# KTH-RPL/cloth-splatting

Measured on AMD Instinct MI355X. Metric: rasterizer fwd+bwd rendered Mpix/s (scene_1, 800x800), higher is better.
Workload: dtype f32

## Files before the change

cloth-splatting_amd/csrc/csplat_raster.hip:

```cpp
#include "csplat_common.h"

#include <atomic>
#include <cstring>
#include <chrono>
#include <mutex>
#include <type_traits>

#include "csplat_raster_math.h"
#include "csplat_raster_k1.h"
#include "csplat_raster_binning.h"
#include "csplat_raster_k5b_k6.h"

namespace {

constexpr int ACC_STRIDE = 16;

#define CSPLAT_ROWMASK_OP(OP, dst, src0, src1, RM)                                                                                  \
    asm("s_nop 1\n\tv_" OP "_f32_dpp %0, %1, %2 quad_perm:[0,1,2,3] row_mask:" RM " bank_mask:0xf" : "+v"(dst) : "v"(src0), "v"(src1))
__device__ __forceinline__ void rows_scan_mul(float f, float Tin, float &Tr, float &Tout) {
    const auto s16 = __builtin_amdgcn_permlane16_swap(__float_as_uint(f), __float_as_uint(f), false, false);
    const float ev = __uint_as_float(s16[0]), od = __uint_as_float(s16[1]);
    const float pr = ev * od;
    const auto s32 = __builtin_amdgcn_permlane32_swap(__float_as_uint(pr), __float_as_uint(pr), false, false);
    const float lo = __uint_as_float(s32[0]), hi = __uint_as_float(s32[1]);
// ... 563 lines not shown
int64_t k7_slots(const csplat_view &w, int tiles) {
    return (w.busy_tiles > 0 && w.num_rendered > 0) ? (int64_t)w.num_rendered / SEG + w.busy_tiles + 1 : max_slots(layout_R(w), tiles);
}
template <typename T>
void fill_list_view(const BinView &b, const ImageView &im, T &k) {
    k.ranges = im.ranges; k.n_contrib = im.n_contrib;
    k.ids_sorted = b.ids_sorted; k.seg_offset = b.seg_offset; k.ckpt = b.ckpt; k.bbits = b.bbits; k.recA = b.recA; k.recB = b.recB;
}
void fill_k7_view(const csplat_view &w, const ScratchView &sv, int tiles, B2View &k, DetView &e) {
    const BinView b = binning_view(w.binning, layout_R(w), tiles);
    const ImageView im = image_view(w.image, w.W, w.H);
    fill_list_view(b, im, k);
    k.final_T = im.final_T; k.slot_tile = b.slot_tile; k.recC = b.recC;
    k.out_color = w.out_color; k.dL_dpix = w.dL_dpix; k.acc = sv.acc; k.R = (uint32_t)layout_R(w); k.det = sv.det;
    if (!sv.det || w.P <= 0) return;
    make_cam(e.cam, w);
    const Geom g = geom_view(w.geom, w.P);
    e.xy = g.xy; e.depth = g.depth; e.radii = w.radii; e.ranges = k.ranges; e.keys_sorted = b.keys_sorted; e.ids_sorted = k.ids_sorted;
    e.det = k.det; e.acc = k.acc;
}

struct Mailboxes {
    volatile uint32_t *host = nullptr;
    uint32_t *dev = nullptr;
    std::atomic<uint32_t> next{1};
    bool tried = false;
};
Mailboxes g_mail;
std::mutex g_mail_mu;
constexpr int MAIL_SLOTS = 64, MAIL_WORDS = 16;

bool mail_init() {
    std::lock_guard<std::mutex> lk(g_mail_mu);
    if (!g_mail.tried) {
        g_mail.tried = true;
        void *h = nullptr, *d = nullptr;
        if (hipHostMalloc(&h, MAIL_SLOTS * MAIL_WORDS * 4, hipHostMallocMapped | hipHostMallocPortable) == hipSuccess &&
            hipHostGetDevicePointer(&d, h, 0) == hipSuccess) {
            memset(h, 0, MAIL_SLOTS * MAIL_WORDS * 4);
            g_mail.host = (volatile uint32_t *)h;
            g_mail.dev = (uint32_t *)d;
        }
        (void)hipGetLastError();
    }
    return g_mail.host != nullptr;
}

unsigned long long *g_stamp_buf = nullptr;
size_t g_stamp_words = 0;
unsigned long long *per_gaussian_stamps(int P) {
    return (g_stamp_buf && g_stamp_words == 8u * ((size_t)cdiv(P, 64) + (size_t)cdiv(P, 32))) ? g_stamp_buf : nullptr;
}

int tsort_mode(int P) { return (P < (1 << 24) ? 1 : 0) | (dbg(CSPLAT_DEBUG_SORT_RADIX_ONLY) ? 2 : 0) | (dbg(CSPLAT_DEBUG_SORT_RADIX_FALLBACK) ? 4 : 0); }

int higher_msb(uint32_t n) {
    int b = 0;
    while ((1u << b) < n && b < 31) b++;
    return b == 0 ? 1 : b;
}

hipEvent_t pooled_event() {
    constexpr int N = 256;
    static hipEvent_t ring[N];
    static std::atomic<unsigned> next{0};
    static std::mutex mu;
    const unsigned k = next.fetch_add(1) % N;
    std::lock_guard<std::mutex> lk(mu);
    if (!ring[k] && hipEventCreateWithFlags(&ring[k], hipEventDisableTiming) != hipSuccess) { (void)hipGetLastError(); return nullptr; }
    return ring[k];
}

}

extern "C" {

int csplat_abi_version(void) { return CSPLAT_ABI_VERSION; }
int csplat_debug_flags(unsigned flags) { g_debug_flags = flags; return 0; }
unsigned csplat_debug_flags_query(void) { return g_debug_flags; }
int csplat_debug_stamps(void *buf, size_t bytes) { g_stamp_buf = (unsigned long long *)buf; g_stamp_words = bytes / 8; return 0; }
}
unsigned long long *csplat_stamp_buffer(size_t need_words) { return (g_stamp_buf && g_stamp_words >= need_words) ? g_stamp_buf : nullptr; }
extern "C" {
const char *csplat_last_error(void) { return g_csplat_err; }

size_t csplat_geom_bytes(int P) { size_t off[G_NFIELDS]; return geom_offsets(P, off); }
size_t csplat_image_bytes(int W, int H) { size_t off[I_NFIELDS]; return image_offsets(W, H, off); }
size_t csplat_binning_bytes(int64_t R, int W, int H) { size_t off[B_NFIELDS]; return binning_offsets(R, tiles_of(W, H), off); }
size_t csplat_temp_bytes(int P, int64_t R, int W, int H) { (void)P; (void)W; (void)H; size_t off[T_NFIELDS]; return temp_offsets(R, off); }
static size_t scratch_bytes(ScratchPath path, int P, int64_t R, int W, int H) {
    size_t off[S_NFIELDS];
    return scratch_offsets(path, P, R, W, H, dbg(CSPLAT_DEBUG_BIT_REPRODUCIBLE), off);
}
size_t csplat_backward_scratch_bytes(int P, int64_t R) { return scratch_bytes(SP_COLOUR, P, R, 0, 0); }
size_t csplat_backward_depth_scratch_bytes(int P, int64_t R, int W, int H) { return scratch_bytes(SP_DEPTH, P, R, W, H); }
size_t csplat_backward_camera_scratch_bytes(int P, int64_t R, int W, int H) { return scratch_bytes(SP_CAMERA, P, R, W, H); }
size_t csplat_backward_feature_scratch_bytes(int P, int64_t R, int W, int H) { return scratch_bytes(SP_FEATURE, P, R, W, H); }
int csplat_geom_layout(int P, size_t *o8) { size_t off[G_NFIELDS]; geom_offsets(P, off); for (int k = 0; k < 8; k++) o8[k] = off[k]; return 0; }
static_assert(B_NFIELDS == 11 && B_KEYS == 0 && B_IDS == 1 && I_RANGES == 0 && I_NCONTRIB == 1 && I_FINALT == 2, "field numbers csplat.h documents");
int csplat_binning_fields(int64_t R, int W, int H, size_t *o11) { binning_offsets(R, tiles_of(W, H), o11); return 0; }
int csplat_binning_layout(int64_t R, int W, int H, size_t *o2) {
    size_t off[B_NFIELDS];
    binning_offsets(R, tiles_of(W, H), off);
    o2[0] = off[B_KEYS]; o2[1] = off[B_IDS];
    return 0;
}
// ... 58 lines not shown
        for (int i = 0; i < MAX_TICKETS && tk < 0; i++)
            if (!g_tickets[i].used) tk = i;
        if (tk >= 0) g_tickets[tk].used = true;
    }
    CSPLAT_REQUIRE(tk >= 0, "csplat_forward_begin: more than 64 forwards begun and not finished");
    FwdTicket &t = g_tickets[tk];
    t.w = w; t.alloc = alloc; t.s = (hipStream_t)w.stream;
    t.cam = cam; t.g = geom_view(gbase, P); t.im = image_view(ibase, W, H); t.gbase = gbase; t.ibase = ibase; t.table = table;
    t.tiles = tiles; t.nb = cdiv(P > 0 ? P : 1, BUCKET_G); t.can_bucket = can_bucket;
    t.use_mail = false; t.tag = 0; t.mb_host = nullptr; t.mb_dev = nullptr;
    if (can_bucket && !dbg(CSPLAT_DEBUG_NO_MAILBOX) && mail_init()) {
        t.use_mail = true;
        t.tag = g_mail.next.fetch_add(1);
        if (t.tag == 0) t.tag = g_mail.next.fetch_add(1);
        const int slot = (int)(t.tag % MAIL_SLOTS);
        t.mb_host = g_mail.host + slot * MAIL_WORDS;
        t.mb_dev = g_mail.dev + slot * MAIL_WORDS;
    }
    *ticket_out = tk;
    return 0;
}

static int nocull_mode() { return dbg(CSPLAT_DEBUG_NO_CULLING) ? 1 : dbg(CSPLAT_DEBUG_CULL_RADIUS_X4) ? 2 : 0; }

static int begin_launch(const FwdTicket &t) {
    hipStream_t s = t.s;
    const csplat_view &w = t.w;
    const int P = w.P, tiles = t.tiles, nb = t.nb;
    if (!t.can_bucket) HIP_TRY(hipMemsetAsync(t.im.ranges, 0, (size_t)tiles * 8, s));
    if (P > 0) {
        ProfScope ps(PROF_K1, s);
        auto form = [&](auto staged) {
            constexpr bool STAGE = decltype(staged)::value;
            auto go = [&](auto kernel) {
                kernel<<<cdiv(P, 256), 256, 0, s>>>(P, w.D, w.M, w.means3D, w.shs, w.colors_precomp, w.opacities, w.scales, w.scale_modifier,
                                                    w.rotations, w.cov3D_precomp, t.cam, t.g, w.radii, nocull_mode());
            };
            if (aa_of(w)) go(k_preprocess_aa<STAGE>);
            else go(k_preprocess<STAGE>);
        };
        if (w.shs != nullptr && w.M == 16 && ((uintptr_t)w.shs & 15u) == 0) form(std::true_type{});
        else form(std::false_type{});
        LAUNCH_CHECK();
    }
    if (t.can_bucket) {
        ProfScope ps(PROF_K2, s);
        if (P > 0) {
            k_tile_count<<<nb, BUCKET_G, (size_t)tiles * 4, s>>>(P, tiles, t.g.xy, w.radii, t.cam, t.table);
            LAUNCH_CHECK();
        } else {
            HIP_TRY(hipMemsetAsync(t.table, 0, (size_t)nb * tiles * 4, s));
        }
        uint32_t *tile_cnt = t.table + (size_t)nb * tiles;
        k_tile_colscan<<<cdiv(tiles, 256), 256, 0, s>>>(tiles, nb, t.table, tile_cnt);
        LAUNCH_CHECK();
        k_tile_scan<<<1, 1024, 0, s>>>(tiles, tile_cnt, t.im.ranges, t.im.info, t.mb_dev, t.tag);
        LAUNCH_CHECK();
    }
    return 0;
}

static bool begin_views_compatible(int V, const int *tk) {
    if (V < 1 || V > RASTER_MAX_VIEWS || dbg(CSPLAT_DEBUG_PER_VIEW_LAUNCHES)) return false;
    const FwdTicket &ta = g_tickets[tk[0]];
    const csplat_view &a = ta.w;
    if (a.P <= 0 || !ta.can_bucket || !a.shs || a.colors_precomp || a.cov3D_precomp || !a.scales || !a.rotations) return false;
    for (int i = 1; i < V; i++) {
        const csplat_view &w = g_tickets[tk[i]].w;
        if (w.P != a.P || w.D != a.D || w.M != a.M || w.W != a.W || w.H != a.H || w.shs != a.shs || w.opacities != a.opacities ||
            w.scales != a.scales || w.scale_modifier != a.scale_modifier || w.colors_precomp || w.cov3D_precomp || !w.rotations ||
            !g_tickets[tk[i]].can_bucket || aa_of(w) != aa_of(a))
            return false;
    }
    return true;
}
static int begin_launch_views(int V, const int *tk, hipStream_t join) {
    const FwdTicket &ta = g_tickets[tk[0]];
    const csplat_view &a = ta.w;
    const int P = a.P, tiles = ta.tiles, nb = ta.nb;
    K1Table tab;
    tab.n = V;
    for (int i = 0; i < V; i++) {
        const FwdTicket &t = g_tickets[tk[i]];
        K1View &k = tab.v[i];
        k.means3D = t.w.means3D; k.rotations = t.w.rotations; k.cam = t.cam; k.g = t.g; k.radii = t.w.radii; k.table = t.table;
        k.info = t.im.info; k.mailbox = t.mb_dev; k.ranges = t.im.ranges; k.tag = t.tag;
    }
    {
        ProfScope ps(PROF_K1, join);
        auto form = [&](auto staged) {
            constexpr bool STAGE = decltype(staged)::value;
            auto go = [&](auto kernel, auto... extra) {
                kernel<<<cdiv(P, K1V_G), 256, 0, join>>>(P, a.D, a.M, a.shs, a.opacities, a.scales, a.scale_modifier, tab, nocull_mode(), extra...);
            };
            if (aa_of(a)) go(k_preprocess_views_aa<STAGE>);
            else if (STAGE && per_gaussian_stamps(P)) go(k_preprocess_views_stamps, per_gaussian_stamps(P));
            else go(k_preprocess_views<STAGE>);
        };
        if (a.M == 16 && ((uintptr_t)a.shs & 15u) == 0) form(std::true_type{});
        else form(std::false_type{});
        LAUNCH_CHECK();
    }
    {
        ProfScope ps(PROF_K2, join);
        k_tile_count_views<<<dim3(nb, V), BUCKET_G, (size_t)tiles * 4, join>>>(P, tiles, tab);
        LAUNCH_CHECK();
        k_tile_colscan_views<<<dim3(cdiv(tiles, 256), V), 256, 0, join>>>(tiles, nb, tab);
        LAUNCH_CHECK();
        k_tile_scan_views<<<V, 1024, 0, join>>>(tiles, nb, tab);
        LAUNCH_CHECK();
    }
    return 0;
}

int csplat_forward_begin(void *stream, int P, int D, int M, const float *bg, int W, int H, const float *means3D,
                         const float *shs, const float *colors_precomp, const float *opacities, const float *scales,
                         float scale_modifier, const float *rotations, const float *cov3D_precomp, const float *view,
                         const float *proj, const float *campos, float tanfovx, float tanfovy, int prefiltered,
                         csplat_alloc_fn alloc, void *alloc_ctx, int32_t *radii, int *ticket_out) {
    CSPLAT_REQUIRE(!(prefiltered & CSPLAT_ANTIALIAS), "csplat_forward / csplat_forward_begin: CSPLAT_ANTIALIAS needs a csplat_view entry point "
                                                      "(csplat_forward_views*), whose backward knows the bit");
    csplat_view w;
    memset(&w, 0, sizeof(w));
    w.stream = stream;
    w.P = P; w.D = D; w.M = M; w.W = W; w.H = H; w.prefiltered = prefiltered;
    w.scale_modifier = scale_modifier; w.tanfovx = tanfovx; w.tanfovy = tanfovy;
    w.bg = bg; w.means3D = means3D; w.shs = shs; w.colors_precomp = colors_precomp; w.opacities = opacities; w.scales = scales;
    w.rotations = rotations; w.cov3D_precomp = cov3D_precomp; w.view = view; w.proj = proj; w.campos = campos;
    w.alloc_ctx = alloc_ctx; w.radii = radii;
    if (int rc = begin_prepare(w, alloc, ticket_out)) return rc;
    const int rc = begin_launch(g_tickets[*ticket_out]);
    if (rc) release_ticket(*ticket_out);
    return rc;
}

static int finish_read(const FwdTicket &t, uint32_t host_info[3], hipStream_t launched_on = nullptr) {
    hipStream_t s = launched_on ? launched_on : t.s;
    host_info[0] = host_info[1] = host_info[2] = 0;
    if (t.can_bucket) {
        bool got = false;
        if (t.use_mail) {
            const auto t0 = std::chrono::steady_clock::now();
            unsigned spins = 0;
            while (!(got = (t.mb_host[2] == t.tag))) {
                if ((++spins & 0x3FFu) == 0 &&
                    std::chrono::duration<double>(std::chrono::steady_clock::now() - t0).count() > 2.0) break;
            }
            if (got) { host_info[0] = t.mb_host[0]; host_info[1] = t.mb_host[1]; host_info[2] = t.mb_host[3]; }
        }
        if (!got) {
            HIP_TRY(hipMemcpyAsync(host_info, t.im.info, 12, hipMemcpyDeviceToHost, s));
            HIP_TRY(hipStreamSynchronize(s));
        }
    } else if (t.w.P > 0) {
        ProfScope ps(PROF_K2, s);
        if (int rc = csplat_inclusive_scan_u32(s, t.g.tiles_touched, t.g.offsets, t.w.P, t.g.scan_tmp)) return rc;
        HIP_TRY(hipMemcpyAsync(host_info, t.g.offsets + (t.w.P - 1), 4, hipMemcpyDeviceToHost, s));
        HIP_TRY(hipStreamSynchronize(s));
        host_info[1] = 0xFFFFFFFFu;
        host_info[2] = 0xFFFFFFFFu;
    }
    CSPLAT_REQUIRE(host_info[0] <= 0x7FFFFFFFu, "csplat_forward: more than 2^31 - 1 tile instances (Gaussian x tile pairs) in one view");
    return 0;
}
#define TSORT_FOR_ITEMS(X) X(2) X(4) X(6) X(8)
static int tsort_items(uint32_t longest) {
    const uint32_t items = (longest + TSORT_THREADS - 1) / TSORT_THREADS;
    return items <= 2 ? 2 : items <= 4 ? 4 : items <= 6 ? 6 : 8;
}
static bool tsort_dense(int items, uint64_t busy) {
    static int s_cus = 0;
    if (s_cus <= 0) {
        int dev = 0;
        if (hipGetDevice(&dev) != hipSuccess || hipDeviceGetAttribute(&s_cus, hipDeviceAttributeMultiprocessorCount, dev) != hipSuccess || s_cus <= 0)
            s_cus = 256;
        (void)hipGetLastError();
    }
    return items <= 6 && 2 * busy > 5 * (uint64_t)s_cus;
}
static uint32_t tile_sort_cap() {
    static int s_lds_big = -1;
    if (s_lds_big < 0) {
        bool ok = true;
#define X(I) ok = ok && hipFuncSetAttribute((const void *)k_tile_sort<I, false>, hipFuncAttributeMaxDynamicSharedMemorySize, 96 * 1024) == hipSuccess && \
                  hipFuncSetAttribute((const void *)k_tile_sort<I, I <= 6>, hipFuncAttributeMaxDynamicSharedMemorySize, 96 * 1024) == hipSuccess &&  \
                  hipFuncSetAttribute((const void *)k_tile_sort_views<I, false>, hipFuncAttributeMaxDynamicSharedMemorySize, 96 * 1024) == hipSuccess && \
                  hipFuncSetAttribute((const void *)k_tile_sort_views<I, I <= 6>, hipFuncAttributeMaxDynamicSharedMemorySize, 96 * 1024) == hipSuccess;
        TSORT_FOR_ITEMS(X)
#undef X
        s_lds_big = ok;
        (void)hipGetLastError();
    }
    return s_lds_big ? (uint32_t)BUCKET_CAP : 5120u;
}
static void tile_sort_launch(hipStream_t s, int tiles, uint32_t longest, uint32_t busy, const ImageView &im, const uint64_t *comp,
                             const BinView &b, int mode) {
    const size_t lds = tsort_lds_bytes((int)longest);
    const int grid = tiles < TSORT_GRID ? tiles : TSORT_GRID, items = tsort_items(longest);
    const bool dense = tsort_dense(items, busy);
    switch (items) {
#define X(I) case I:                                                                                                                        \
// ... 87 lines not shown
    bool park(const csplat_view *key, const Caps &caps) {
        std::lock_guard<std::mutex> lk(g_pending_mu);
        for (PendingViews &p : g_pending)
            if (!p.parked) {
                p.parked = true; p.key = key; p.V = n; p.caps = caps;
                for (int i = 0; i < n; i++) p.tk[i] = tk[i];
                n = handed = 0;
                return true;
            }
        return false;
    }
    void adopt(const PendingViews &p) {
        for (n = 0; n < p.V; n++) tk[n] = p.tk[n];
    }
};
}

static bool p2_qualifies(int V, const int *tk) {
    if (V < 1 || V > RASTER_MAX_VIEWS || dbg(CSPLAT_DEBUG_PER_VIEW_LAUNCHES)) return false;
    const FwdTicket &a = g_tickets[tk[0]];
    for (int i = 0; i < V; i++) {
        const FwdTicket &t = g_tickets[tk[i]];
        if (!t.can_bucket || t.w.P != a.w.P || t.w.W != a.w.W || t.w.H != a.w.H || t.w.P <= 0) return false;
    }
    return true;
}

static int p2_launch(int V, const int *tk, csplat_view *v, hipStream_t join, const Caps &caps, int spec, uint32_t *valid) {
    const FwdTicket &a = g_tickets[tk[0]];
    const int P = a.w.P, W = a.w.W, H = a.w.H, tiles = a.tiles, nb = a.nb;
    const uint32_t Lcap = caps.longest, Bcap = caps.busy;
    P2Table tab;
    tab.valid = valid; tab.nviews = V;
    uint32_t maxR = 0;
    for (int i = 0; i < V; i++) {
        const FwdTicket &t = g_tickets[tk[i]];
        const uint32_t R = caps.R[i];
        maxR = R > maxR ? R : maxR;
        void *bbase = t.alloc(t.w.alloc_ctx, CSPLAT_CHUNK_BINNING, csplat_binning_bytes(R, W, H));
        void *tbase = t.alloc(t.w.alloc_ctx, CSPLAT_CHUNK_TEMP, csplat_temp_bytes(P, R, W, H));
        CSPLAT_REQUIRE(bbase && tbase, "allocator returned NULL");
        const BinView b = binning_view(bbase, R, tiles);
        P2View &k = tab.v[i];
        k.g = t.g; k.cam = t.cam; k.radii = t.w.radii; k.table = t.table; k.ranges = t.im.ranges;
        k.keys_u = temp_view(tbase, R).keys_u;
        k.keys_sorted = b.keys_sorted; k.ids_sorted = b.ids_sorted; k.seg_offset = b.seg_offset; k.slot_tile = b.slot_tile;
        k.ckpt = b.ckpt; k.mask16 = b.mask16; k.bbits = b.bbits; k.bmask = b.bmask; k.recA = b.recA; k.recB = b.recB; k.recC = b.recC;
        k.bg = t.w.bg; k.final_T = t.im.final_T; k.n_contrib = t.im.n_contrib; k.out_color = v[i].out_color; k.out_depth = v[i].out_depth;
        k.R = R; k.info = t.im.info; k.Lcap = Lcap; k.Bcap = Bcap; k.spec = spec;
        v[i].layout_rendered = (int)R; v[i].geom = t.gbase; v[i].binning = bbase; v[i].image = t.ibase;
    }
    {
        ProfScope ps(PROF_K3, join);
        k_emit_bucket_views<<<dim3(nb + 1, V), BUCKET_G, (size_t)tiles * 4, join>>>(P, tiles, tab);
        LAUNCH_CHECK();
    }
    {
        ProfScope ps(PROF_K4, join);
        tile_sort_views_launch(join, tiles, V, Lcap, Bcap, tab, tsort_mode(P));
        LAUNCH_CHECK();
    }
    {
        ProfScope ps(PROF_K5, join);
        const int exact = dbg(DBG_NO_ELLIPSE_STAGE) ? 0 : 1, nbm = cdiv((int64_t)maxR + 1, 256);
        if (V == 1 || V == 2 || V == 4 || V == 8)
            k_block_masks_views<<<dim3((unsigned)(((int64_t)nbm * V + 7) / 8 * 8)), 256, 0, join>>>(tab, exact, V);
        else
            k_block_masks_views<<<dim3(nbm, V), 256, 0, join>>>(tab, exact, 0);
        LAUNCH_CHECK();
    }
    {
        ProfScope ps(PROF_K6, join);
        const int total = cdiv(tiles, 8) * 128, bg_ = cdiv((int)Bcap, 8) * 128, busy_grid = bg_ < total ? bg_ : total;
        if (!dbg(CSPLAT_DEBUG_K6_ROWS))
            k_composite_fwd_views<false><<<dim3(busy_grid + K6_EXTRA, V), 64, 0, join>>>(tiles, W, H, tab, busy_grid);
        else
            k_composite_fwd_views<true><<<dim3(busy_grid + K6_EXTRA, V), 64, 0, join>>>(tiles, W, H, tab, busy_grid);
        LAUNCH_CHECK();
    }
    return 0;
}

enum P2Result { P2_DONE, P2_PER_VIEW };
static int p2_settle(int V, const int *tk, csplat_view *v, hipStream_t join, const Caps *speculated, int *relaunched, P2Result *how) {
    const csplat_view &a = g_tickets[tk[0]].w;
    *how = P2_PER_VIEW;
    uint32_t info[RASTER_MAX_VIEWS][3];
    for (int i = 0; i < V; i++)
        if (int rc = finish_read(g_tickets[tk[i]], info[i], join)) return rc;
    auto accept = [&]() {
        for (int i = 0; i < V; i++) { v[i].num_rendered = (int)info[i][0]; v[i].busy_tiles = (int)info[i][2]; }
        *how = P2_DONE;
    };
    if (speculated) {
        bool fits = true;
        for (int i = 0; i < V; i++)
            fits = fits && info[i][0] - 1u < speculated->R[i] && info[i][1] <= speculated->longest && info[i][2] <= speculated->busy;
        remember(a.P, a.W, a.H, V, info);
        if (fits) { accept(); return 0; }
    }
    const uint32_t cap = tile_sort_cap();
    Caps exact;
    exact.longest = exact.busy = 0;
    for (int i = 0; i < V; i++) {
        if (info[i][1] > cap || info[i][0] == 0) return 0;
        exact.longest = info[i][1] > exact.longest ? info[i][1] : exact.longest;
        exact.busy = info[i][2] > exact.busy ? info[i][2] : exact.busy;
// ... 843 lines not shown
```

cloth-splatting_amd/csrc/csplat_raster_binning.h:

```cpp
#pragma once

namespace {

__global__ __launch_bounds__(256) void k_emit_keys(int P, const float2 *__restrict__ xy, const float *__restrict__ depth,
                                                    const uint32_t *__restrict__ offsets,
                                                    const int32_t *__restrict__ radii, Cam cam,
                                                    uint64_t *__restrict__ keys, uint32_t *__restrict__ ids) {
    const int i = blockIdx.x * blockDim.x + threadIdx.x;
    if (i >= P) return;
    const int rad = radii[i];
    if (rad <= 0) return;
    uint32_t off = (i == 0) ? 0u : offsets[i - 1];
    const float2 p = xy[i];
    int minx, miny, maxx, maxy;
    tile_rect(p.x, p.y, rad, cam, minx, miny, maxx, maxy);
    const uint32_t dbits = __float_as_uint(depth[i]);
    for (int y = miny; y < maxy; y++)
        for (int x = minx; x < maxx; x++) {
            keys[off] = ((uint64_t)(uint32_t)(y * cam.gx + x) << 32) | dbits;
            ids[off] = (uint32_t)i;
            off++;
        }
}

__global__ __launch_bounds__(256) void k_tile_ranges(int64_t R, const uint64_t *__restrict__ keys, int2 *__restrict__ ranges) {
    const int64_t i = (int64_t)blockIdx.x * blockDim.x + threadIdx.x;
    if (i >= R) return;
    const uint32_t t = (uint32_t)(keys[i] >> 32);
    if (i == 0) ranges[t].x = 0;
    else {
        const uint32_t tp = (uint32_t)(keys[i - 1] >> 32);
        if (tp != t) { ranges[tp].y = (int)i; ranges[t].x = (int)i; }
    }
    if (i == R - 1) ranges[t].y = (int)R;
}

constexpr int BUCKET_CAP = 8192;
constexpr int BUCKET_TILES = 12288;
constexpr int BUCKET_G = 1024;

__device__ __forceinline__ void tile_count_body(int P, int tiles, const float2 *__restrict__ xy,
                                                const int32_t *__restrict__ radii, const Cam &cam,
                                                uint32_t *__restrict__ table) {
    extern __shared__ uint32_t s_hist[];
    for (int t = threadIdx.x; t < tiles; t += BUCKET_G) s_hist[t] = 0u;
    __syncthreads();
    const int i = blockIdx.x * BUCKET_G + threadIdx.x;
    if (i < P) {
        const int rad = radii[i];
        if (rad > 0) {
            const float2 p = xy[i];
            int minx, miny, maxx, maxy;
            tile_rect(p.x, p.y, rad, cam, minx, miny, maxx, maxy);
            for (int y = miny; y < maxy; y++)
                for (int x = minx; x < maxx; x++) atomicAdd(&s_hist[y * cam.gx + x], 1u);
        }
    }
    __syncthreads();
    uint32_t *row = table + (size_t)blockIdx.x * tiles;
    for (int t = threadIdx.x; t < tiles; t += BUCKET_G) row[t] = s_hist[t];
}
__global__ __launch_bounds__(BUCKET_G) void k_tile_count(int P, int tiles, const float2 *__restrict__ xy,
                                                          const int32_t *__restrict__ radii, Cam cam,
                                                          uint32_t *__restrict__ table) {
    tile_count_body(P, tiles, xy, radii, cam, table);
}
__global__ __launch_bounds__(BUCKET_G) void k_tile_count_views(int P, int tiles, K1Table tab) {
    const K1View &w = tab.v[blockIdx.y];
    tile_count_body(P, tiles, w.g.xy, w.radii, w.cam, w.table);
}

__device__ __forceinline__ void tile_colscan_body(int tiles, int nb, uint32_t *__restrict__ table, uint32_t *__restrict__ cnt) {
    const int t = blockIdx.x * 256 + threadIdx.x;
    if (t >= tiles) return;
    uint32_t run = 0;
    int b = 0;
    for (; b + 8 <= nb; b += 8) {
        uint32_t v[8];
#pragma unroll
        for (int u = 0; u < 8; u++) v[u] = table[(size_t)(b + u) * tiles + t];
#pragma unroll
        for (int u = 0; u < 8; u++) { table[(size_t)(b + u) * tiles + t] = run; run += v[u]; }
    }
    for (; b < nb; b++) { const uint32_t v = table[(size_t)b * tiles + t]; table[(size_t)b * tiles + t] = run; run += v; }
    cnt[t] = run;
}
__global__ __launch_bounds__(256) void k_tile_colscan(int tiles, int nb, uint32_t *__restrict__ table, uint32_t *__restrict__ cnt) {
    tile_colscan_body(tiles, nb, table, cnt);
}
__global__ __launch_bounds__(256) void k_tile_colscan_views(int tiles, int nb, K1Table tab) {
    uint32_t *table = tab.v[blockIdx.y].table;
    tile_colscan_body(tiles, nb, table, table + (size_t)nb * tiles);
}

constexpr int INFO_BUSY = 64;
constexpr int LPT_BINS = 512;
constexpr int TSCAN_ITEMS = BUCKET_TILES / 1024;
__device__ __forceinline__ void tile_scan_body(int tiles, const uint32_t *__restrict__ cnt, int2 *__restrict__ ranges,
                                               uint32_t *__restrict__ info, volatile uint32_t *mailbox, uint32_t tag) {
    __shared__ unsigned long long s_w[17];
    __shared__ uint32_t s_max[16];
    __shared__ uint32_t s_bin[LPT_BINS + 1];
    const int lane = threadIdx.x & 63, w = threadIdx.x >> 6;
    uint32_t *busy = info + INFO_BUSY;
    uint32_t *lpt = busy + tiles + 4;
    const int per = (tiles + 1023) / 1024, t0 = threadIdx.x * per;
    uint32_t c[TSCAN_ITEMS];
#pragma unroll
    for (int k = 0; k < TSCAN_ITEMS; k++) c[k] = (k < per && t0 + k < tiles) ? cnt[t0 + k] : 0u;
    for (int i = threadIdx.x; i <= LPT_BINS; i += 1024) s_bin[i] = 0u;
    uint32_t mx = 0;
    unsigned long long v0 = 0ull;
#pragma unroll
    for (int k = 0; k < TSCAN_ITEMS; k++) { mx = max(mx, c[k]); v0 += (unsigned long long)c[k] | ((unsigned long long)(c[k] ? 1u : 0u) << 32); }
    unsigned long long inc = v0;
#pragma unroll
    for (int d = 1; d < 64; d <<= 1) { const unsigned long long o = __shfl_up(inc, d, 64); if (lane >= d) inc += o; }
    if (lane == 63) s_w[w] = inc;
    __syncthreads();
    if (w == 0) {
        unsigned long long v = lane < 16 ? s_w[lane] : 0ull, vi = v;
#pragma unroll
        for (int d = 1; d < 16; d <<= 1) { const unsigned long long o = __shfl_up(vi, d, 64); if (lane >= d) vi += o; }
        if (lane < 16) s_w[lane] = vi - v;
        if (lane == 15) s_w[16] = vi;
    }
    __syncthreads();
    const unsigned long long carry = s_w[16];
    {
        unsigned long long exl = s_w[w] + inc - v0;
#pragma unroll
        for (int k = 0; k < TSCAN_ITEMS; k++) {
            const int t = t0 + k;
            if (k < per && t < tiles) {
                const uint32_t ex = (uint32_t)exl, nz = (uint32_t)(exl >> 32);
                ranges[t] = c[k] ? make_int2((int)ex, (int)(ex + c[k])) : make_int2(0, 0);
                if (c[k]) {
                    busy[1 + nz] = (uint32_t)t;
                    atomicAdd(&s_bin[LPT_BINS - 1 - min(c[k] >> 4, (uint32_t)(LPT_BINS - 1))], 1u);
                } else {
                    lpt[tiles - 1 - (t - (int)nz)] = (uint32_t)t;
                }
                exl += (unsigned long long)c[k] | ((unsigned long long)(c[k] ? 1u : 0u) << 32);
            }
        }
    }
    __syncthreads();
    {
        if (w == 0) {
            uint32_t v[LPT_BINS / 64], run = 0;
#pragma unroll
            for (int k = 0; k < LPT_BINS / 64; k++) { v[k] = s_bin[lane * (LPT_BINS / 64) + k]; run += v[k]; }
            uint32_t binc = run;
#pragma unroll
            for (int d = 1; d < 64; d <<= 1) { const uint32_t o = (uint32_t)__shfl_up((int)binc, d, 64); if (lane >= d) binc += o; }
            uint32_t base = binc - run;
#pragma unroll
            for (int k = 0; k < LPT_BINS / 64; k++) { s_bin[lane * (LPT_BINS / 64) + k] = base; base += v[k]; }
        }
        __syncthreads();
#pragma unroll
        for (int k = 0; k < TSCAN_ITEMS; k++)
            if (c[k]) lpt[atomicAdd(&s_bin[LPT_BINS - 1 - min(c[k] >> 4, (uint32_t)(LPT_BINS - 1))], 1u)] = (uint32_t)(t0 + k);
    }
#pragma unroll
    for (int d = 32; d > 0; d >>= 1) mx = max(mx, (uint32_t)__shfl_xor((int)mx, d, 64));
    if (lane == 0) s_max[w] = mx;
    __syncthreads();
    if (threadIdx.x == 0) {
        uint32_t m = 0;
        for (int k = 0; k < 16; k++) m = max(m, s_max[k]);
        info[0] = (uint32_t)carry;
        info[1] = m;
        info[2] = (uint32_t)(carry >> 32);
        busy[0] = (uint32_t)(carry >> 32);
        if (mailbox) {
            mailbox[0] = (uint32_t)carry;
            mailbox[1] = m;
            mailbox[3] = (uint32_t)(carry >> 32);
            __threadfence_system();
            mailbox[2] = tag;
        }
    }
}
__global__ __launch_bounds__(1024) void k_tile_scan(int tiles, const uint32_t *__restrict__ cnt, int2 *__restrict__ ranges,
                                                     uint32_t *__restrict__ info, volatile uint32_t *mailbox, uint32_t tag) {
    tile_scan_body(tiles, cnt, ranges, info, mailbox, tag);
}
__global__ __launch_bounds__(1024) void k_tile_scan_views(int tiles, int nb, K1Table tab) {
    const K1View &w = tab.v[blockIdx.x];
    tile_scan_body(tiles, w.table + (size_t)nb * tiles, w.ranges, w.info, w.mailbox, w.tag);
}

__device__ __forceinline__ void emit_bucket_body(int P, int tiles, const float2 *__restrict__ xy,
                                                 const float *__restrict__ depth, const int32_t *__restrict__ radii,
                                                 const Cam &cam, const uint32_t *__restrict__ table,
                                                 const int2 *__restrict__ ranges, uint64_t *__restrict__ comp) {
    extern __shared__ uint32_t s_base[];
    const uint32_t *row = table + (size_t)blockIdx.x * tiles;
    for (int t = threadIdx.x; t < tiles; t += BUCKET_G) s_base[t] = (uint32_t)ranges[t].x + row[t];
    __syncthreads();
    const int i = blockIdx.x * BUCKET_G + threadIdx.x;
    if (i >= P) return;
    const int rad = radii[i];
    if (rad <= 0) return;
    const float2 p = xy[i];
    int minx, miny, maxx, maxy;
    tile_rect(p.x, p.y, rad, cam, minx, miny, maxx, maxy);
    const uint64_t v = ((uint64_t)__float_as_uint(depth[i]) << 32) | (uint32_t)i;
    for (int y = miny; y < maxy; y++)
        for (int x = minx; x < maxx; x++) comp[atomicAdd(&s_base[y * cam.gx + x], 1u)] = v;
}
__global__ __launch_bounds__(BUCKET_G) void k_emit_bucket(int P, int tiles, const float2 *__restrict__ xy,
                                                           const float *__restrict__ depth, const int32_t *__restrict__ radii,
                                                           Cam cam, const uint32_t *__restrict__ table,
                                                           const int2 *__restrict__ ranges, uint64_t *__restrict__ comp) {
    emit_bucket_body(P, tiles, xy, depth, radii, cam, table, ranges, comp);
}

struct P2View {
    Geom g;
    Cam cam;
    const int32_t *radii;
    const uint32_t *table;
    int2 *ranges;
    uint64_t *keys_u, *keys_sorted;
    uint32_t *ids_sorted;
    int *seg_offset, *slot_tile;
    float4 *ckpt;
    uint16_t *mask16;
    unsigned long long *bbits;
    unsigned long long *bmask;
    float4 *recA, *recB;
    float2 *recC;
    const float *bg;
    float *final_T;
    uint32_t *n_contrib;
    float *out_color, *out_depth;
    uint32_t R;
    const uint32_t *info;
    uint32_t Lcap;
    uint32_t Bcap;
    int spec;
};
struct P2Table { P2View v[RASTER_MAX_VIEWS]; uint32_t *valid; int nviews; };
__device__ __forceinline__ bool p2_live(const P2View &w) { return !w.spec || (w.info[0] - 1u < w.R && w.info[1] <= w.Lcap && w.info[2] <= w.Bcap); }
__device__ __forceinline__ void seg_plan_body(int tiles, const int2 *__restrict__ ranges, int *__restrict__ seg_offset,
                                              int *__restrict__ slot_tile);
__global__ __launch_bounds__(BUCKET_G) void k_emit_bucket_views(int P, int tiles, P2Table tab) {
    const P2View &w = tab.v[blockIdx.y];
    if (!p2_live(w)) return;
    if (blockIdx.x == gridDim.x - 1) { seg_plan_body(tiles, w.ranges, w.seg_offset, w.slot_tile); return; }
    emit_bucket_body(P, tiles, w.g.xy, w.g.depth, w.radii, w.cam, w.table, w.ranges, w.keys_u);
}

constexpr int TSORT_THREADS = 1024;
constexpr int TSORT_WAVES = TSORT_THREADS / 64;
constexpr int TSORT_NB = 4 * TSORT_THREADS;
constexpr int TSORT_GRID = 512;
constexpr int TSORT_LONG = 64;
constexpr int TSORT_WORDS = TSORT_NB + 4 + 256 + 8 + 2 + 2 + TSORT_WAVES + 2;
__host__ __device__ inline size_t tsort_lds_bytes(int longest) {
    const int items = (longest > 0 ? longest : 1) + TSORT_THREADS - 1;
    return (size_t)(items / TSORT_THREADS) * TSORT_THREADS * 8 + (size_t)TSORT_WORDS * 4;
}

template <int ITEMS>
__device__ __forceinline__ void tile_sort_body(const int2 *__restrict__ ranges, const uint64_t *__restrict__ comp,
                                               uint64_t *__restrict__ keys_sorted,
                                               uint32_t *__restrict__ ids_sorted, int mode, int tile) {
    extern __shared__ uint64_t s_key[];
    const int2 r = ranges[tile];
    const int n = r.y - r.x;
    if (n <= 0) return;
    const int skip_byte3 = mode & 1;
    const int items = (n + TSORT_THREADS - 1) / TSORT_THREADS;
    uint32_t *s_cnt = reinterpret_cast<uint32_t *>(s_key + (size_t)items * TSORT_THREADS);
    uint32_t *s_dig = s_cnt + TSORT_NB + 4;
    int lane = threadIdx.x & 63, w = threadIdx.x >> 6;
    asm volatile("" : "+v"(lane), "+v"(w));
    const int wbase = w * items * 64;
    const uint64_t lt = (1ull << lane) - 1ull;
    uint64_t key[ITEMS];
    uint32_t rank[ITEMS];
#pragma unroll
    for (int i = 0; i < ITEMS; i++) {
        const int idx = wbase + i * 64 + lane;
        key[i] = (i < items && idx < n) ? comp[r.x + idx] : ~0ull;
    }
    uint32_t *s_diff = s_dig + 264;
    uint32_t *s_mm = s_diff + 2;
    uint32_t *s_wtot = s_mm + 2;
    const uint64_t hi = (uint64_t)(uint32_t)tile << 32;
    if (!(mode & 2)) {
        uint32_t dmin = ~0u, dmax = 0u;
#pragma unroll
        for (int i = 0; i < ITEMS; i++) {
            const int idx = wbase + i * 64 + lane;
            if (i < items && idx < n) { const uint32_t d = (uint32_t)(key[i] >> 32); dmin = min(dmin, d); dmax = max(dmax, d); }
        }
#pragma unroll
        for (int o = 32; o > 0; o >>= 1) {
            dmin = min(dmin, (uint32_t)__shfl_xor((int)dmin, o, 64));
            dmax = max(dmax, (uint32_t)__shfl_xor((int)dmax, o, 64));
        }
        if (threadIdx.x == 0) { s_mm[0] = ~0u; s_mm[1] = 0u; }
        reinterpret_cast<uint4 *>(s_cnt)[threadIdx.x] = make_uint4(0u, 0u, 0u, 0u);
// ... 310 lines not shown
```

Baseline: 4826.

## Split tile column scan across waves and pack mailbox words with tags

The per-tile column prefix scan over bucket rows changes from one thread per tile walking all rows serially to 16 waves that each scan a slice of rows, then combine partial sums through shared memory. The host mailbox now stores three 64-bit words, each carrying the tag in its high half, instead of four 32-bit words followed by a system fence. This removes the fence and lets the host check arrival with three relaxed loads. The change also adds optional timestamp-instrumented variants of the binning kernels, which stay inactive unless a stamp buffer of matching size has been set up.

Result: no change. 4831, median of 3 (+0.1%).

```diff
diff --git a/cloth-splatting_amd/csrc/csplat_raster.hip b/cloth-splatting_amd/csrc/csplat_raster.hip
--- a/cloth-splatting_amd/csrc/csplat_raster.hip
+++ b/cloth-splatting_amd/csrc/csplat_raster.hip
@@ -639,6 +639,17 @@
     return (g_stamp_buf && g_stamp_words == 8u * ((size_t)cdiv(P, 64) + (size_t)cdiv(P, 32))) ? g_stamp_buf : nullptr;
 }
 
+struct BinStamps { unsigned long long *count, *colscan, *scan, *emit; };
+bool binning_stamps(int tiles, int nb, int V, BinStamps &b) {
+    const size_t n_count = (size_t)nb * V, n_col = (size_t)cdiv(tiles, CS_COLS) * V, n_scan = (size_t)V, n_emit = (size_t)(nb + 1) * V;
+    if (!g_stamp_buf || g_stamp_words != (n_count + n_col + n_scan + n_emit) * BIN_STAMP_WORDS) return false;
+    b.count = g_stamp_buf;
+    b.colscan = b.count + n_count * BIN_STAMP_WORDS;
+    b.scan = b.colscan + n_col * BIN_STAMP_WORDS;
+    b.emit = b.scan + n_scan * BIN_STAMP_WORDS;
+    return true;
+}
+
 int tsort_mode(int P) { return (P < (1 << 24) ? 1 : 0) | (dbg(CSPLAT_DEBUG_SORT_RADIX_ONLY) ? 2 : 0) | (dbg(CSPLAT_DEBUG_SORT_RADIX_FALLBACK) ? 4 : 0); }
 
 int higher_msb(uint32_t n) {
@@ -803,7 +814,7 @@
             HIP_TRY(hipMemsetAsync(t.table, 0, (size_t)nb * tiles * 4, s));
         }
         uint32_t *tile_cnt = t.table + (size_t)nb * tiles;
-        k_tile_colscan<<<cdiv(tiles, 256), 256, 0, s>>>(tiles, nb, t.table, tile_cnt);
+        k_tile_colscan<<<cdiv(tiles, CS_COLS), CS_WAVES * 64, 0, s>>>(tiles, nb, t.table, tile_cnt);
         LAUNCH_CHECK();
         k_tile_scan<<<1, 1024, 0, s>>>(tiles, tile_cnt, t.im.ranges, t.im.info, t.mb_dev, t.tag);
         LAUNCH_CHECK();
@@ -854,11 +865,16 @@
     }
     {
         ProfScope ps(PROF_K2, join);
-        k_tile_count_views<<<dim3(nb, V), BUCKET_G, (size_t)tiles * 4, join>>>(P, tiles, tab);
+        BinStamps st;
+        const bool stamped = binning_stamps(tiles, nb, V, st);
+        if (stamped) k_tile_count_views_stamps<<<dim3(nb, V), BUCKET_G, (size_t)tiles * 4, join>>>(P, tiles, tab, st.count);
+        else k_tile_count_views<<<dim3(nb, V), BUCKET_G, (size_t)tiles * 4, join>>>(P, tiles, tab);
         LAUNCH_CHECK();
-        k_tile_colscan_views<<<dim3(cdiv(tiles, 256), V), 256, 0, join>>>(tiles, nb, tab);
+        if (stamped) k_tile_colscan_views_stamps<<<dim3(cdiv(tiles, CS_COLS), V), CS_WAVES * 64, 0, join>>>(tiles, nb, tab, st.colscan);
+        else k_tile_colscan_views<<<dim3(cdiv(tiles, CS_COLS), V), CS_WAVES * 64, 0, join>>>(tiles, nb, tab);
         LAUNCH_CHECK();
-        k_tile_scan_views<<<V, 1024, 0, join>>>(tiles, nb, tab);
+        if (stamped) k_tile_scan_views_stamps<<<V, 1024, 0, join>>>(tiles, nb, tab, st.scan);
+        else k_tile_scan_views<<<V, 1024, 0, join>>>(tiles, nb, tab);
         LAUNCH_CHECK();
     }
     return 0;
@@ -893,11 +909,17 @@
         if (t.use_mail) {
             const auto t0 = std::chrono::steady_clock::now();
             unsigned spins = 0;
-            while (!(got = (t.mb_host[2] == t.tag))) {
+            const volatile uint64_t *mb = (const volatile uint64_t *)t.mb_host;
+            uint64_t m[3];
+            auto arrived = [&]() {
+                for (int k = 0; k < 3; k++) m[k] = __atomic_load_n(mb + k, __ATOMIC_RELAXED);
+                return (uint32_t)(m[0] >> 32) == t.tag && (uint32_t)(m[1] >> 32) == t.tag && (uint32_t)(m[2] >> 32) == t.tag;
+            };
+            while (!(got = arrived())) {
                 if ((++spins & 0x3FFu) == 0 &&
                     std::chrono::duration<double>(std::chrono::steady_clock::now() - t0).count() > 2.0) break;
             }
-            if (got) { host_info[0] = t.mb_host[0]; host_info[1] = t.mb_host[1]; host_info[2] = t.mb_host[3]; }
+            if (got) { host_info[0] = (uint32_t)m[0]; host_info[1] = (uint32_t)m[1]; host_info[2] = (uint32_t)m[2]; }
         }
         if (!got) {
             HIP_TRY(hipMemcpyAsync(host_info, t.im.info, 12, hipMemcpyDeviceToHost, s));
@@ -1091,7 +1113,9 @@
     }
     {
         ProfScope ps(PROF_K3, join);
-        k_emit_bucket_views<<<dim3(nb + 1, V), BUCKET_G, (size_t)tiles * 4, join>>>(P, tiles, tab);
+        BinStamps st;
+        if (binning_stamps(tiles, nb, V, st)) k_emit_bucket_views_stamps<<<dim3(nb + 1, V), BUCKET_G, (size_t)tiles * 4, join>>>(P, tiles, tab, st.emit);
+        else k_emit_bucket_views<<<dim3(nb + 1, V), BUCKET_G, (size_t)tiles * 4, join>>>(P, tiles, tab);
         LAUNCH_CHECK();
     }
     {
diff --git a/cloth-splatting_amd/csrc/csplat_raster_binning.h b/cloth-splatting_amd/csrc/csplat_raster_binning.h
--- a/cloth-splatting_amd/csrc/csplat_raster_binning.h
+++ b/cloth-splatting_amd/csrc/csplat_raster_binning.h
@@ -38,18 +38,25 @@
 constexpr int BUCKET_CAP = 8192;
 constexpr int BUCKET_TILES = 12288;
 constexpr int BUCKET_G = 1024;
-
+constexpr int CS_COLS = 64;
+constexpr int CS_WAVES = 16;
+
+template <class MK = NoMark>
 __device__ __forceinline__ void tile_count_body(int P, int tiles, const float2 *__restrict__ xy,
                                                 const int32_t *__restrict__ radii, const Cam &cam,
-                                                uint32_t *__restrict__ table) {
+                                                uint32_t *__restrict__ table, const MK &mark = MK()) {
     extern __shared__ uint32_t s_hist[];
+    mark(0, 0.f);
     for (int t = threadIdx.x; t < tiles; t += BUCKET_G) s_hist[t] = 0u;
     __syncthreads();
+    mark(1, 0.f);
     const int i = blockIdx.x * BUCKET_G + threadIdx.x;
     if (i < P) {
         const int rad = radii[i];
+        mark(2, __int_as_float(rad));
         if (rad > 0) {
             const float2 p = xy[i];
+            mark(3, p.x);
             int minx, miny, maxx, maxy;
             tile_rect(p.x, p.y, rad, cam, minx, miny, maxx, maxy);
             for (int y = miny; y < maxy; y++)
@@ -57,8 +64,10 @@
         }
     }
     __syncthreads();
+    mark(4, 0.f);
     uint32_t *row = table + (size_t)blockIdx.x * tiles;
     for (int t = threadIdx.x; t < tiles; t += BUCKET_G) row[t] = s_hist[t];
+    mark(5, 0.f);
 }
 __global__ __launch_bounds__(BUCKET_G) void k_tile_count(int P, int tiles, const float2 *__restrict__ xy,
                                                           const int32_t *__restrict__ radii, Cam cam,
@@ -69,38 +78,108 @@
     const K1View &w = tab.v[blockIdx.y];
     tile_count_body(P, tiles, w.g.xy, w.radii, w.cam, w.table);
 }
-
-__device__ __forceinline__ void tile_colscan_body(int tiles, int nb, uint32_t *__restrict__ table, uint32_t *__restrict__ cnt) {
-    const int t = blockIdx.x * 256 + threadIdx.x;
-    if (t >= tiles) return;
+constexpr int BIN_STAMP_WORDS = 16;
+__device__ __forceinline__ StampMark bin_stamp_mark(unsigned long long *buf) {
+    return StampMark{buf + ((size_t)blockIdx.y * gridDim.x + blockIdx.x) * BIN_STAMP_WORDS};
+}
+__global__ __launch_bounds__(BUCKET_G) void k_tile_count_views_stamps(int P, int tiles, K1Table tab, unsigned long long *stamp_buf) {
+    const K1View &w = tab.v[blockIdx.y];
+    tile_count_body(P, tiles, w.g.xy, w.radii, w.cam, w.table, bin_stamp_mark(stamp_buf));
+}
+
+constexpr int CS_BATCH = 16;
+__device__ __forceinline__ uint32_t colscan_base(uint32_t *s_tot, int g, int lane, uint32_t run) {
+    s_tot[g * CS_COLS + lane] = run;
+    __syncthreads();
+    uint32_t base = 0;
+    const int gu = __builtin_amdgcn_readfirstlane(g);
+    for (int k = 0; k < gu; k++) base += s_tot[k * CS_COLS + lane];
+    return base;
+}
+template <int B, class MK>
+__device__ __forceinline__ void colscan_rows(int tiles, int nb, int r, uint32_t *__restrict__ table, uint32_t *__restrict__ cnt,
+                                             uint32_t *s_tot, const MK &mark) {
+    const int lane = threadIdx.x & 63, g = threadIdx.x >> 6, t = blockIdx.x * CS_COLS + lane, tc = min(t, tiles - 1);
+    const int b0 = g * r, b1 = min(nb, b0 + r);
+    uint32_t v[B];
+#pragma unroll
+    for (int u = 0; u < B; u++) v[u] = table[(size_t)min(b0 + u, nb - 1) * tiles + tc];
+    mark(1, __uint_as_float(v[B - 1]));
     uint32_t run = 0;
-    int b = 0;
-    for (; b + 8 <= nb; b += 8) {
-        uint32_t v[8];
-#pragma unroll
-        for (int u = 0; u < 8; u++) v[u] = table[(size_t)(b + u) * tiles + t];
-#pragma unroll
-        for (int u = 0; u < 8; u++) { table[(size_t)(b + u) * tiles + t] = run; run += v[u]; }
-    }
-    for (; b < nb; b++) { const uint32_t v = table[(size_t)b * tiles + t]; table[(size_t)b * tiles + t] = run; run += v; }
-    cnt[t] = run;
-}
-__global__ __launch_bounds__(256) void k_tile_colscan(int tiles, int nb, uint32_t *__restrict__ table, uint32_t *__restrict__ cnt) {
+#pragma unroll
+    for (int u = 0; u < B; u++) { const uint32_t x = b0 + u < b1 ? v[u] : 0u; v[u] = run; run += x; }
+    const uint32_t base = colscan_base(s_tot, g, lane, run);
+    mark(2, 0.f);
+    if (t < tiles) {
+#pragma unroll
+        for (int u = 0; u < B; u++)
+            if (b0 + u < b1) table[(size_t)(b0 + u) * tiles + t] = base + v[u];
+        if (g == CS_WAVES - 1) cnt[t] = base + run;
+    }
+    mark(3, 0.f);
+}
+template <class MK>
+__device__ __forceinline__ void colscan_long(int tiles, int nb, int r, uint32_t *__restrict__ table, uint32_t *__restrict__ cnt,
+                                             uint32_t *s_tot, const MK &mark) {
+    const int lane = threadIdx.x & 63, g = threadIdx.x >> 6, t = blockIdx.x * CS_COLS + lane, tc = min(t, tiles - 1);
+    const int b0 = g * r, b1 = min(nb, b0 + r);
+    uint32_t run = 0;
+    for (int b = b0; b < b1; b += CS_BATCH) {
+        uint32_t v[CS_BATCH];
+#pragma unroll
+        for (int u = 0; u < CS_BATCH; u++) v[u] = table[(size_t)min(b + u, b1 - 1) * tiles + tc];
+        if (b == b0) mark(1, __uint_as_float(v[CS_BATCH - 1]));
+#pragma unroll
+        for (int u = 0; u < CS_BATCH; u++) run += b + u < b1 ? v[u] : 0u;
+    }
+    uint32_t acc = colscan_base(s_tot, g, lane, run);
+    mark(2, 0.f);
+    if (g == CS_WAVES - 1 && t < tiles) cnt[t] = acc + run;
+    for (int b = b0; b < b1; b += CS_BATCH) {
+        uint32_t v[CS_BATCH];
+#pragma unroll
+        for (int u = 0; u < CS_BATCH; u++) v[u] = table[(size_t)min(b + u, b1 - 1) * tiles + tc];
+#pragma unroll
+        for (int u = 0; u < CS_BATCH; u++)
+            if (b + u < b1) {
+                if (t < tiles) table[(size_t)(b + u) * tiles + t] = acc;
+                acc += v[u];
+            }
+    }
+    mark(3, 0.f);
+}
+template <class MK = NoMark>
+__device__ __forceinline__ void tile_colscan_body(int tiles, int nb, uint32_t *__restrict__ table, uint32_t *__restrict__ cnt, const MK &mark = MK()) {
+    __shared__ uint32_t s_tot[CS_WAVES * CS_COLS];
+    mark(0, 0.f);
+    const int r = (nb + CS_WAVES - 1) / CS_WAVES;
+    if (r <= 4) colscan_rows<4>(tiles, nb, r, table, cnt, s_tot, mark);
+    else if (r <= 8) colscan_rows<8>(tiles, nb, r, table, cnt, s_tot, mark);
+    else if (r <= CS_BATCH) colscan_rows<CS_BATCH>(tiles, nb, r, table, cnt, s_tot, mark);
+    else colscan_long(tiles, nb, r, table, cnt, s_tot, mark);
+}
+__global__ __launch_bounds__(CS_WAVES * 64) void k_tile_colscan(int tiles, int nb, uint32_t *__restrict__ table, uint32_t *__restrict__ cnt) {
     tile_colscan_body(tiles, nb, table, cnt);
 }
-__global__ __launch_bounds__(256) void k_tile_colscan_views(int tiles, int nb, K1Table tab) {
+__global__ __launch_bounds__(CS_WAVES * 64) void k_tile_colscan_views(int tiles, int nb, K1Table tab) {
     uint32_t *table = tab.v[blockIdx.y].table;
     tile_colscan_body(tiles, nb, table, table + (size_t)nb * tiles);
+}
+__global__ __launch_bounds__(CS_WAVES * 64) void k_tile_colscan_views_stamps(int tiles, int nb, K1Table tab, unsigned long long *stamp_buf) {
+    uint32_t *table = tab.v[blockIdx.y].table;
+    tile_colscan_body(tiles, nb, table, table + (size_t)nb * tiles, bin_stamp_mark(stamp_buf));
 }
 
 constexpr int INFO_BUSY = 64;
 constexpr int LPT_BINS = 512;
 constexpr int TSCAN_ITEMS = BUCKET_TILES / 1024;
+template <class MK = NoMark>
 __device__ __forceinline__ void tile_scan_body(int tiles, const uint32_t *__restrict__ cnt, int2 *__restrict__ ranges,
-                                               uint32_t *__restrict__ info, volatile uint32_t *mailbox, uint32_t tag) {
+                                               uint32_t *__restrict__ info, volatile uint32_t *mailbox, uint32_t tag, const MK &mark = MK()) {
     __shared__ unsigned long long s_w[17];
     __shared__ uint32_t s_max[16];
     __shared__ uint32_t s_bin[LPT_BINS + 1];
+    mark(0, 0.f);
     const int lane = threadIdx.x & 63, w = threadIdx.x >> 6;
     uint32_t *busy = info + INFO_BUSY;
     uint32_t *lpt = busy + tiles + 4;
@@ -109,6 +188,7 @@
 #pragma unroll
     for (int k = 0; k < TSCAN_ITEMS; k++) c[k] = (k < per && t0 + k < tiles) ? cnt[t0 + k] : 0u;
     for (int i = threadIdx.x; i <= LPT_BINS; i += 1024) s_bin[i] = 0u;
+    mark(1, __uint_as_float(c[0]));
     uint32_t mx = 0;
     unsigned long long v0 = 0ull;
 #pragma unroll
@@ -118,6 +198,7 @@
     for (int d = 1; d < 64; d <<= 1) { const unsigned long long o = __shfl_up(inc, d, 64); if (lane >= d) inc += o; }
     if (lane == 63) s_w[w] = inc;
     __syncthreads();
+    mark(2, 0.f);
     if (w == 0) {
         unsigned long long v = lane < 16 ? s_w[lane] : 0ull, vi = v;
 #pragma unroll
@@ -126,6 +207,7 @@
         if (lane == 15) s_w[16] = vi;
     }
     __syncthreads();
+    mark(3, 0.f);
     const unsigned long long carry = s_w[16];
     {
         unsigned long long exl = s_w[w] + inc - v0;
@@ -146,6 +228,7 @@
         }
     }
     __syncthreads();
+    mark(4, 0.f);
     {
         if (w == 0) {
             uint32_t v[LPT_BINS / 64], run = 0;
@@ -159,6 +242,7 @@
             for (int k = 0; k < LPT_BINS / 64; k++) { s_bin[lane * (LPT_BINS / 64) + k] = base; base += v[k]; }
         }
         __syncthreads();
+        mark(5, 0.f);
 #pragma unroll
         for (int k = 0; k < TSCAN_ITEMS; k++)
             if (c[k]) lpt[atomicAdd(&s_bin[LPT_BINS - 1 - min(c[k] >> 4, (uint32_t)(LPT_BINS - 1))], 1u)] = (uint32_t)(t0 + k);
@@ -167,6 +251,7 @@
     for (int d = 32; d > 0; d >>= 1) mx = max(mx, (uint32_t)__shfl_xor((int)mx, d, 64));
     if (lane == 0) s_max[w] = mx;
     __syncthreads();
+    mark(6, 0.f);
     if (threadIdx.x == 0) {
         uint32_t m = 0;
         for (int k = 0; k < 16; k++) m = max(m, s_max[k]);
@@ -174,13 +259,15 @@
         info[1] = m;
         info[2] = (uint32_t)(carry >> 32);
         busy[0] = (uint32_t)(carry >> 32);
+        mark(7, 0.f);
         if (mailbox) {
-            mailbox[0] = (uint32_t)carry;
-            mailbox[1] = m;
-            mailbox[3] = (uint32_t)(carry >> 32);
-            __threadfence_system();
-            mailbox[2] = tag;
-        }
+            unsigned long long *mb = (unsigned long long *)mailbox;
+            const unsigned long long hi = (unsigned long long)tag << 32;
+            __hip_atomic_store(mb + 0, hi | (uint32_t)carry, __ATOMIC_RELAXED, __HIP_MEMORY_SCOPE_SYSTEM);
+            __hip_atomic_store(mb + 1, hi | m, __ATOMIC_RELAXED, __HIP_MEMORY_SCOPE_SYSTEM);
+            __hip_atomic_store(mb + 2, hi | (uint32_t)(carry >> 32), __ATOMIC_RELAXED, __HIP_MEMORY_SCOPE_SYSTEM);
+        }
+        mark(8, 0.f);
     }
 }
 __global__ __launch_bounds__(1024) void k_tile_scan(int tiles, const uint32_t *__restrict__ cnt, int2 *__restrict__ ranges,
@@ -191,25 +278,35 @@
     const K1View &w = tab.v[blockIdx.x];
     tile_scan_body(tiles, w.table + (size_t)nb * tiles, w.ranges, w.info, w.mailbox, w.tag);
 }
-
+__global__ __launch_bounds__(1024) void k_tile_scan_views_stamps(int tiles, int nb, K1Table tab, unsigned long long *stamp_buf) {
+    const K1View &w = tab.v[blockIdx.x];
+    tile_scan_body(tiles, w.table + (size_t)nb * tiles, w.ranges, w.info, w.mailbox, w.tag, bin_stamp_mark(stamp_buf));
+}
+
+template <class MK = NoMark>
 __device__ __forceinline__ void emit_bucket_body(int P, int tiles, const float2 *__restrict__ xy,
                                                  const float *__restrict__ depth, const int32_t *__restrict__ radii,
                                                  const Cam &cam, const uint32_t *__restrict__ table,
-                                                 const int2 *__restrict__ ranges, uint64_t *__restrict__ comp) {
+                                                 const int2 *__restrict__ ranges, uint64_t *__restrict__ comp, const MK &mark = MK()) {
     extern __shared__ uint32_t s_base[];
+    mark(0, 0.f);
     const uint32_t *row = table + (size_t)blockIdx.x * tiles;
     for (int t = threadIdx.x; t < tiles; t += BUCKET_G) s_base[t] = (uint32_t)ranges[t].x + row[t];
     __syncthreads();
+    mark(1, 0.f);
     const int i = blockIdx.x * BUCKET_G + threadIdx.x;
     if (i >= P) return;
     const int rad = radii[i];
+    mark(2, __int_as_float(rad));
     if (rad <= 0) return;
     const float2 p = xy[i];
     int minx, miny, maxx, maxy;
     tile_rect(p.x, p.y, rad, cam, minx, miny, maxx, maxy);
     const uint64_t v = ((uint64_t)__float_as_uint(depth[i]) << 32) | (uint32_t)i;
+    mark(3, __uint_as_float((uint32_t)(v >> 32) ^ (uint32_t)minx));
     for (int y = miny; y < maxy; y++)
         for (int x = minx; x < maxx; x++) comp[atomicAdd(&s_base[y * cam.gx + x], 1u)] = v;
+    mark(4, 0.f);
 }
 __global__ __launch_bounds__(BUCKET_G) void k_emit_bucket(int P, int tiles, const float2 *__restrict__ xy,
                                                            const float *__restrict__ depth, const int32_t *__restrict__ radii,
@@ -253,6 +350,12 @@
     if (blockIdx.x == gridDim.x - 1) { seg_plan_body(tiles, w.ranges, w.seg_offset, w.slot_tile); return; }
     emit_bucket_body(P, tiles, w.g.xy, w.g.depth, w.radii, w.cam, w.table, w.ranges, w.keys_u);
 }
+__global__ __launch_bounds__(BUCKET_G) void k_emit_bucket_views_stamps(int P, int tiles, P2Table tab, unsigned long long *stamp_buf) {
+    const P2View &w = tab.v[blockIdx.y];
+    if (!p2_live(w)) return;
+    if (blockIdx.x == gridDim.x - 1) { seg_plan_body(tiles, w.ranges, w.seg_offset, w.slot_tile); return; }
+    emit_bucket_body(P, tiles, w.g.xy, w.g.depth, w.radii, w.cam, w.table, w.ranges, w.keys_u, bin_stamp_mark(stamp_buf));
+}
 
 constexpr int TSORT_THREADS = 1024;
 constexpr int TSORT_WAVES = TSORT_THREADS / 64;
```
